# shayneobrien/generative-models

Measured on AMD Instinct MI355X. Metric: images/sec (28x28 MNIST) per D+G step, NSGAN bs=256, higher is better.
Workload: dtype f32; 1 GPU; NSGAN MNIST bs=256 fp32 per GPU (BASELINE.json configs[1]); 784-400-20 MLPs, N=50000 synthetic Bernoulli images, parity-mode RNG protocol, Adam 2e-4, D_steps=1; global_batch=256, parallelism=dp1, ranks_seen=1, gradient_exchange=none (1 rank), timing=one 2064-step timed region, cold_start_inclusive=False

## Files before the change

generative_models_amd/_lib.py:

```python
import ctypes
import os
from ctypes import POINTER, c_char_p, c_float, c_int, c_int32, c_int64, c_void_p

HERE = os.path.dirname(os.path.abspath(__file__))
LIB_PATH = os.environ.get("GM_LIB_PATH") or os.path.join(HERE, "libgm_hip.so")

GM_EINVAL = -10001
ACT_ID, ACT_RELU, ACT_SIGMOID = 0, 1, 2
ACT = {"id": ACT_ID, None: ACT_ID, "relu": ACT_RELU, "sigmoid": ACT_SIGMOID}
LOSS = {"ns": 0, "mm": 1, "w": 2, "ls": 3, "ra": 4, "fisher": 5, "f_total_variation": 6,
        "f_forward_kl": 7, "f_reverse_kl": 8, "f_pearson": 9, "f_hellinger": 10,
        "f_jensen_shannon": 11}


class Slot(ctypes.Structure):
    _fields_ = [("ctr", c_void_p), ("mul", c_int32), ("add", c_int32), ("ring", c_int32),
                ("stride", c_int64)]


def slot(ctr=0, mul=0, add=0, ring=0, stride=0):
    return Slot(ctr or None, mul, add, ring, stride)


NO_SLOT = Slot(None, 0, 0, 0, 0)
# ... 145 lines not shown
    "gm_version": (c_int, []),
    "gm_arch": (c_char_p, []),
    "gm_last_error": (c_char_p, []),
    "gm_tick": (c_int, [_P, _P, c_int64]),
    "gm_copy_slot_f32": (c_int, [_P, _P, Slot, _P, Slot, c_int64]),
    "gm_gather_rows": (c_int, [_P, _P, c_int64, _P, Slot, _P, c_int64, c_int, c_int]),
    "gm_linear_fwd": (c_int, [_P, _P, c_int64, Slot, _P, _P, _P, c_int64, c_int, c_int, c_int,
                              c_int]),
    "gm_linear_bwd_dx": (c_int, [_P, _P, c_int64, _P, _P, c_int64, _P, c_int64, c_int, c_int,
                                 c_int, c_int]),
    "gm_linear_bwd_dw": (c_int, [_P, _P, c_int64, _P, c_int64, Slot, _P, _P, c_int, c_int, c_int,
                                 c_int]),
    "gm_linear_fwd_ex": (c_int, [_P, POINTER(FwdArgs)]),
    "gm_linear_bwd_dx_ex": (c_int, [_P, POINTER(DxArgs)]),
    "gm_linear_bwd_dw_ex": (c_int, [_P, POINTER(DwAdamArgs), POINTER(DwAdamArgs), POINTER(DwTail)]),
    "gm_gan_loss": (c_int, [_P, c_int, c_int, _P, _P, c_int, c_int, POINTER(c_float), c_int,
                            c_float, _P, Slot, _P, _P, _P, _P]),
    "gm_gan_loss_phase": (c_int, [_P, c_int, c_int, _P, _P, c_int, c_int, POINTER(c_float), c_int,
                                  c_float, _P, Slot, _P, _P, _P, _P, c_int, _P, c_float]),
    "gm_l1_rows_dp": (c_int, [_P, _P, c_int64, _P, c_int64, c_int, c_int, c_int, c_int, _P, _P, c_int64, _P]),
    "gm_began_dloss_dp": (c_int, [_P, _P, c_int, c_int, _P, _P, Slot]),
    "gm_std_sums": (c_int, [_P, _P, c_int64, c_int, c_int, _P, _P]),
    "gm_std_from_sums": (c_int, [_P, _P, c_int64, _P]),
    "gm_adam": (c_int, [_P, _P, _P, _P, _P, c_int64, _P, Slot, ctypes.c_double, ctypes.c_double,
                        ctypes.c_double, ctypes.c_double, c_float]),
    "gm_interp": (c_int, [_P, _P, Slot, _P, c_int64, _P, c_int64, _P, c_int64, c_int, c_int]),
    "gm_gp_u": (c_int, [_P, _P, _P, c_int64, _P, _P, c_int64, c_int, c_int]),
    "gm_gp_norm": (c_int, [_P, _P, c_int64, _P, c_int64, _P, c_float, c_float, c_float, c_int,
                           c_int]),
    "gm_gp_dw2": (c_int, [_P, _P, _P, c_int64, _P, c_int64, _P, c_int, c_int]),
# ... 165 lines not shown
```

generative_models_amd/csrc/gm_gemm.hip:

```cpp
#include "gm_common.h"
#include "gm_head.h"
#include "gm_gather.h"
#include "gm_dvae.h"
#include "gm_ldsdma.h"

#include <cstdlib>
#include <type_traits>

typedef float f32x16 __attribute__((ext_vector_type(16)));

#ifdef GM_STAMPS
namespace gm_stamps {
constexpr int WAVES = 16, IDS = 40, HDR = 8, MAXB = 512, SLOT_WORDS = HDR + 2 * MAXB + WAVES * IDS * 2, SLOTS = 64;
static unsigned long long* host_buf = nullptr;
static int host_tile = 0, host_next = 0;
struct Ctx { unsigned long long* slot; int tile; };
__device__ __forceinline__ void rec(const Ctx& c, int tile, int id) {
    if (!c.slot || tile != c.tile || (threadIdx.x & 63)) return;
    __builtin_amdgcn_sched_barrier(0);
    unsigned long long* w = c.slot + HDR + 2 * MAXB + ((threadIdx.x >> 6) * IDS + id) * 2;
    w[0] = clock64(); w[1] = wall_clock64();
    __builtin_amdgcn_sched_barrier(0);
}
__device__ __forceinline__ void edge(const Ctx& c, bool exit_, int tile, int M, int N, int K, int mode) {
// ... 23 lines not shown
#define GM_STAMP_EDGE(p, exit_, tile, mode) do {} while (0)
#define GM_STAMP_AFTER(v) do {} while (0)
#endif

namespace {

constexpr int TM = 32, TN = 32;

enum { MODE_FWD = 0, MODE_DX = 1, MODE_DW = 2 };

struct GemmP {
    const float* A;
    const float* B;
    float* C;
    int M, N, K;
    int64_t lda, ldb, ldc;
    const float* bias;
    const float* aux;
    int64_t ldaux;
    float* db;
    int ones_from;
    int n_real;
    int epi;
    int accumulate;
    gm_slot a_slot, b_slot;
    int tn;
    int lds_tm, lds_mpx;
    int dma;
    int vec_epi;
    const float* ip_eps; gm_slot ip_slot;
    const float* ip_x; int64_t ip_ldx;
    float* ip_out; int64_t ip_ldo;
    int ip_rows;
    gm_adam_epi adam;
    const float* hd_w2; const float* hd_b2; float* hd_part; int64_t hd_ldp; float* hd_snap;
    const float* sq_x; int64_t sq_ldx; float* sq_dA; int64_t sq_lda; float* sq_part; int64_t sq_ldp;
    const float* rp_ml; int64_t rp_ldml; const float* rp_eps; gm_slot rp_slot; float* rp_dml; int64_t rp_ldd;
    int rp_Z;
    const float* fold_w2;
    const float* add;
    int64_t ldadd;
// ... 41 lines not shown
                                         int kb, int K) {
    const float* col = P + min(x, X - 1);
    return make_float4(col[(int64_t)min(kb + 0, K - 1) * ld], col[(int64_t)min(kb + 1, K - 1) * ld],
                       col[(int64_t)min(kb + 2, K - 1) * ld], col[(int64_t)min(kb + 3, K - 1) * ld]);
}
__device__ __forceinline__ float4 fix_xc(float4 v, int x, int X, int kb, int K, int ones_col,
                                         int ones_from = 0) {
    const bool okx = x < X, oc = (x == ones_col);
    v.x = (kb + 0 < K) ? (okx ? v.x : ((oc && kb + 0 >= ones_from) ? 1.f : 0.f)) : 0.f;
    v.y = (kb + 1 < K) ? (okx ? v.y : ((oc && kb + 1 >= ones_from) ? 1.f : 0.f)) : 0.f;
    v.z = (kb + 2 < K) ? (okx ? v.z : ((oc && kb + 2 >= ones_from) ? 1.f : 0.f)) : 0.f;
    v.w = (kb + 3 < K) ? (okx ? v.w : ((oc && kb + 3 >= ones_from) ? 1.f : 0.f)) : 0.f;
    return v;
}

__device__ __forceinline__ float fwd_value(const GemmP& p, float v, int n) {
    if (p.bias) v += p.bias[n];
    if (p.epi == GM_ACT_RELU) v = fmaxf(v, 0.f);
    else if (p.epi == GM_ACT_SIGMOID) v = gm_sigmoid(v);
    return v;
}

template <int MODE, bool LBL = false>
__device__ __forceinline__ void store_element(const GemmP& p, float v, int m, int n, float* kept = nullptr) {
    if (MODE == MODE_FWD) {
        if constexpr (LBL) v += p.lb_E[(int64_t)n * p.lb_C + gm_row_label(p.lb, m, p.lb_C)];
        v = fwd_value(p, v, n);
        p.C[(int64_t)m * p.ldc + n] = v;
        if (p.ip_out && m < p.ip_rows) {
            const float ev = (p.ip_eps + gm_slot_offset(p.ip_slot))[m];
// ... 567 lines not shown
#pragma unroll
                for (int f = 0; f < NI; ++f)
#pragma unroll
                    for (int r = 0; r < 4; ++r) {
                        const int row = MI * (4 * g4 + r) + e, col = NI * i16 + f;
                        if ((row >> 5) == bm && (col >> 5) == bnk)
                            red[red_idx(w, row & 31, col & 31)] = acc[e][f][r];
                    }
            __syncthreads();
            reduce_and_store<MODE_DW, WAVES, (MI > 1 ? 32 : 16)>(p, red, t, m0 + 32 * bm, n0 + 32 * bnk,
                                                                 (2 * bnk + 1 < NI) ? 0x7fffffff : n0 + 32 * bnk + 16,
                                                                 (2 * bm + 1 < MI) ? 32 : 16);
        }
}

template <int MI, int NI, bool OF, int FOLD, bool SL>
__device__ __forceinline__ void gemm16_dw_dma(const GemmP& p, float* red, int bx, int by, float* sds,
                                              const FoldP* fold, int gx) {
    constexpr int WAVES = 16, NP = MI + NI, CH = NP * 256;
    if (gx > 0) {
        const int gy = (p.M + 16 * MI - 1) / (16 * MI), total = gx * gy;
        const int L = by * gx + bx, x = L & 7, k = L >> 3;
        const int base = total >> 3, rem = total & 7;
        const int T = x * base + min(x, rem) + k;
        by = T % gy; bx = T / gy;
    }
    const int t = threadIdx.x, lane = t & 63;
    const int w = __builtin_amdgcn_readfirstlane(t >> 6);
    const int i16 = lane & 15, g4 = lane >> 4;
    const int m0 = by * (16 * MI), n0 = bx * (16 * NI);
#ifdef GM_STAMPS
    const gm_stamps::Ctx st_slot = p.stamp; const int st_tile = by * max(gx, 1) + bx;
#endif
    GM_STAMP_EDGE(p, false, st_tile, MODE_DW + 20);
    GM_STAMP(st_slot, st_tile, 0);
    const int b_cols = p.n_real;
    const int ones_col = p.db ? p.n_real : -1;
    const int nchunks = (p.K + 15) >> 4;
    float* buf = red + w * CH;
    const uint32_t buf_b = (uint32_t)(uintptr_t)buf;
    const int am = m0 + MI * i16, bn = n0 + NI * i16;

    const float* src[NP]; int srow[NP], sld[NP];
#pragma unroll
    for (int j = 0; j < NP; ++j) {
        const bool isA = j < MI;
        const int idx = (isA ? j : j - MI) * 64 + lane;
        const int row = isA ? idx / (4 * MI) : idx / (4 * NI);
        const int c4 = isA ? idx % (4 * MI) : idx % (4 * NI);
        const int col = isA ? min(m0 + 4 * c4, p.M - 4) : min(n0 + 4 * c4, b_cols - 4);
        src[j] = (isA ? slot_base<SL>(p.A, p.a_slot) : slot_base<SL>(p.B, p.b_slot)) + col;
        sld[j] = isA ? (int)p.lda : (int)p.ldb;
        srow[j] = row;
    }
    auto issue = [&](int c) {
#pragma unroll
        for (int j = 0; j < NP; ++j) {
            const int k = min(16 * c + srow[j], p.K - 1);
            slab::glds16(src[j] + (int64_t)k * sld[j], buf_b + j * 1024u);
        }
    };

    float fw[FOLD == 1 ? MI : 1];
    if constexpr (FOLD == 1) {
#pragma unroll
        for (int e = 0; e < MI; ++e) fw[e] = (am + e < p.M) ? p.fold_w2[min(am + e, p.M - 1)] : 0.f;
    }
// ... 58 lines not shown
    GM_STAMP(st_slot, st_tile, 9);
    dw_il_reduce<MI, NI>(p, red, acc, m0, n0, true);
    GM_STAMP(st_slot, st_tile, 12);
    GM_STAMP_EDGE(p, true, st_tile, MODE_DW + 20);
}

template <int MODE, bool DMA, int MI, int NI> struct RedSize {
    static constexpr int base = 16 * 32 * 32;
    static constexpr int onepass = (MODE == MODE_DW && MI * NI > 4) ? 16 * 256 * MI * NI : 0;
    static constexpr int dma = (MODE == MODE_DW && DMA) ? 16 * (MI + NI) * 256 : 0;
    static constexpr int m1 = base > onepass ? base : onepass;
    static constexpr int value = m1 > dma ? m1 : dma;
};

template <int MODE, bool VEC, int WAVES, int G, bool XV, int MI, int NI, bool OF = false, int FOLD = 0, bool DMA = false,
          bool TP = false, bool PK = false, bool SL = true, bool LBL = false>
__device__ __forceinline__ void gemm16_body(const GemmP& p, float* red, int bx, int by,
                                            float* sds = nullptr, const FoldP* fold = nullptr, int gx = 0,
                                            float* kept = nullptr) {
    static_assert(!TP || (FOLD == 1 && !DMA), "two-phase losses: folded weight gradient, operands through registers");
    static_assert(FOLD == 0 || (FOLD == 1 && MODE == MODE_DW && XV) || (FOLD == 2 && MODE == MODE_DX && VEC),
                  "folded head: 16-byte operand paths only");
    static_assert(G == 1, "per-chunk schedule (G stays in the kernel names so that they keep their shape across rounds)");
    static_assert(!PK || (WAVES == 16 && !DMA && ((MODE == MODE_FWD && VEC) || (MODE == MODE_DW && XV))),
                  "bit-packed operand rows: 16-byte operand paths through registers only");
    if constexpr (DMA && MODE == MODE_DW && XV && WAVES == 16 && FOLD != 2) {
        gemm16_dw_dma<MI, NI, OF, FOLD, SL>(p, red, bx, by, sds, fold, gx);
        return;
    }
    const int t = threadIdx.x;
    const int lane = t & 63, w = t >> 6;
    const int i16 = lane & 15, g4 = lane >> 4;
    const int m0 = by * (16 * MI), n0 = bx * (16 * NI);
#ifdef GM_STAMPS
    const gm_stamps::Ctx st_slot = p.stamp; const int st_tile = by * (int)gridDim.x + bx;
#endif
    GM_STAMP_EDGE(p, false, st_tile, MODE);
    GM_STAMP(st_slot, st_tile, 0);

    const float* A = slot_base<SL>(p.A, p.a_slot);
    const float* B = slot_base<SL>(p.B, p.b_slot);
    const int b_cols = (MODE == MODE_DW) ? p.n_real : p.N;
    const int ones_col = (MODE == MODE_DW && p.db) ? p.n_real : -1;
    const int nchunks = (p.K + 15) >> 4;
    GM_STAMP_AFTER(A); GM_STAMP_AFTER(B); GM_STAMP_AFTER(nchunks);
    GM_STAMP(st_slot, st_tile, 16);

    float4 fw[FOLD == 1 ? MI : 1];
    float fds[FOLD == 2 ? MI : 1];
    const int xq_ld = lane & 3, xe_ld = (lane >> 2) & 3;
    constexpr bool XMAP_A = MODE == MODE_DW && XV, XMAP_B = MODE != MODE_FWD && XV;
    const int ia = XMAP_A ? sigma16(i16) : i16, ib = XMAP_B ? sigma16(i16) : i16;
    if constexpr (FOLD == 1) {
#pragma unroll
        for (int mi = 0; mi < MI; ++mi)
            fw[mi] = *reinterpret_cast<const float4*>(
                p.fold_w2 + min(m0 + 16 * mi + 4 * xq_ld, p.M - 4));
    }
    auto load_a = [&](int c, int mi) -> float4 {
        const int kb = 16 * c + 4 * g4, x0 = m0 + 16 * mi;
        if (MODE == MODE_DW) {
            if (XV) return raw_xc4_16(A, p.lda, x0, p.M, c, p.K, lane);
            return raw_xc(A, p.lda, x0 + i16, p.M, kb, p.K);
        }
        return raw_kc<VEC>(A, p.lda, x0 + i16, p.M, kb, p.K);
    };
    auto load_b = [&](int c, int ni) -> float4 {
        const int kb = 16 * c + 4 * g4, x0 = n0 + 16 * ni;
        if (MODE == MODE_FWD) return raw_kc<VEC>(B, p.ldb, x0 + i16, p.N, kb, p.K);
        if (XV) return raw_xc4_16(B, p.ldb, x0, b_cols, c, p.K, lane);
        return raw_xc(B, p.ldb, x0 + i16, b_cols, kb, p.K);
    };
    auto fix_a = [&](float4 v, int c, int mi, float4 wk) -> float4 {
        const int kb = 16 * c + 4 * g4, x = m0 + 16 * mi + ia;
        if constexpr (FOLD == 1)
            v = fold_dh4(v, sds[min(16 * c + 4 * g4 + xe_ld, p.K - 1)], fw[mi]);
        if constexpr (FOLD == 2) v = fold_dh4(v, fds[mi], wk);
        if (MODE == MODE_DW)
            return fix_xc(XV ? lane48_transpose(v, lane) : v, x, p.M, kb, p.K, -1);
        return fix_kc(v, x, p.M, kb, p.K);
    };
    auto fix_b = [&](float4 v, int c, int ni) -> float4 {
        const int kb = 16 * c + 4 * g4, x = n0 + 16 * ni + ib;
        if (MODE == MODE_FWD) return fix_kc(v, x, p.N, kb, p.K);
        return fix_xc(XV ? lane48_transpose(v, lane) : v, x, b_cols, kb, p.K, ones_col, OF ? p.ones_from : 0);
    };

    f32x4 acc[MI][NI];
#pragma unroll
    for (int mi = 0; mi < MI; ++mi)
#pragma unroll
        for (int ni = 0; ni < NI; ++ni) acc[mi][ni] = f32x4{0.f, 0.f, 0.f, 0.f};

    const int nq = (nchunks - w + WAVES - 1) / WAVES;
    auto consume = [&](const float4 (&ra)[MI], const float4 (&rb)[NI], float4 wk, int q) {
        const int cq = w + q * WAVES;
        float4 fa[MI], fb[NI];
#pragma unroll
        for (int mi = 0; mi < MI; ++mi) fa[mi] = fix_a(ra[mi], cq, mi, wk);
#pragma unroll
        for (int ni = 0; ni < NI; ++ni) fb[ni] = fix_b(rb[ni], cq, ni);
        GM_STAMP_AFTER(fa[MI - 1].x); GM_STAMP_AFTER(fb[NI - 1].x);
        if (q < 4) GM_STAMP(st_slot, st_tile, 1 + 2 * q);
#pragma unroll
        for (int mi = 0; mi < MI; ++mi)
#pragma unroll
            for (int ni = 0; ni < NI; ++ni) {
                f32x4 c4 = acc[mi][ni];
                c4 = __builtin_amdgcn_mfma_f32_16x16x4f32(fa[mi].x, fb[ni].x, c4, 0, 0, 0);
                c4 = __builtin_amdgcn_mfma_f32_16x16x4f32(fa[mi].y, fb[ni].y, c4, 0, 0, 0);
// ... 33 lines not shown
            }
        } else if constexpr (FOLD == 2) {
            if (t < 16 * MI) {
                float s_, ds_, l_;
                fold_row(*fold, min(m0 + t, fold->R - 1), s_, ds_, l_);
                sds[t] = ds_;
            }
            GM_STAMP(st_slot, st_tile, 15);
            __syncthreads();
#pragma unroll
            for (int mi = 0; mi < MI; ++mi) fds[mi] = sds[16 * mi + i16];
        }
    };
    if constexpr (PK) {
        constexpr int PN = MODE == MODE_FWD ? MI : NI;
        auto pk_elem = [&](int c, int j) -> int {
            return MODE == MODE_FWD ? min(16 * c + 4 * g4, p.K - 4) : min(n0 + 16 * j + 4 * xq_ld, b_cols - 4);
        };
        auto load_pk = [&](int c, int j) -> uint32_t {
            const int row = MODE == MODE_FWD ? m0 + 16 * j + i16 : 16 * c + 4 * g4 + xe_ld;
            return p.pk_bits[(int64_t)row * p.pk_wpr + (pk_elem(c, j) >> 5)];
        };
        const int nq_s = __builtin_amdgcn_readfirstlane(nq);
        int q_pk;
        if (MODE == MODE_FWD) q_pk = (m0 < p.pk_rows) ? nq_s : 0;
        else q_pk = min(nq_s, max(0, ((p.pk_rows >> 4) - __builtin_amdgcn_readfirstlane(w) + WAVES - 1) / WAVES));
        auto do_chunk = [&](auto is_pk, auto with_prologue, int q) {
            constexpr bool P = decltype(is_pk)::value;
            float4 ra[MI], rb[NI];
            uint32_t pw[PN];
// ... 38 lines not shown
        float4 pv[4];
        if constexpr (FOLD == 1 && !TP) {
            if (t < fold->R) fold_part_load(*fold, t, pv);
        }
        if constexpr (FOLD == 2) {
            if (t < 16 * MI) fold_part_load(*fold, min(m0 + t, fold->R - 1), pv);
        }
        if (have) {
#pragma unroll
            for (int mi = 0; mi < MI; ++mi) ra[mi] = load_a(w, mi);
#pragma unroll
            for (int ni = 0; ni < NI; ++ni) rb[ni] = load_b(w, ni);
            wk = load_wk(w);
        }
        GM_STAMP(st_slot, st_tile, 17);
        if constexpr (FOLD == 1 && !TP) fold_fill_lds_pre(*fold, sds, fold->R, pv);
        else if constexpr (FOLD == 2) {
            if (t < 16 * MI) {
                float s_, ds_, l_;
                fold_row_of(*fold, min(m0 + t, fold->R - 1), fold_score_of(*fold, pv), s_, ds_, l_);
                sds[t] = ds_;
            }
            GM_STAMP(st_slot, st_tile, 15);
            __syncthreads();
#pragma unroll
            for (int mi = 0; mi < MI; ++mi) fds[mi] = sds[16 * mi + i16];
        }
        else fold_prologue();
        GM_STAMP(st_slot, st_tile, 13);
        if (have) consume(ra, rb, wk, 0);
        q_first = 1;
    }
    for (int q = q_first; q < nq; ++q) {
        float4 ra[MI], rb[NI];
        const int cc = w + q * WAVES;
#pragma unroll
        for (int mi = 0; mi < MI; ++mi) ra[mi] = load_a(cc, mi);
#pragma unroll
        for (int ni = 0; ni < NI; ++ni) rb[ni] = load_b(cc, ni);
        const float4 wk = load_wk(cc);
        consume(ra, rb, wk, q);
    }
    }
    GM_STAMP(st_slot, st_tile, 9);
    if constexpr (MODE == MODE_DW && WAVES == 16 && MI * NI > 4) {
// ... 26 lines not shown
            if (bm + bn == 0) GM_STAMP(st_slot, st_tile, 10);
            reduce_and_store<MODE, WAVES, (MI > 1 ? 32 : 16), LBL>(p, red, t, m0 + 32 * bm, n0 + 32 * bn,
                                                              (2 * bn + 1 < NI) ? 0x7fffffff : n0 + 32 * bn + 16,
                                                              (2 * bm + 1 < MI) ? 32 : 16,
                                                              kept ? kept + 32 * bm * KEEP_LD + 32 * bn : nullptr);
        }
    GM_STAMP(st_slot, st_tile, 12);
    GM_STAMP_EDGE(p, true, st_tile, MODE);
}

template <int MODE, bool VEC, int WAVES, int G, bool XV, int MI, int NI, bool DMA = false, bool SL = false>
__global__ __launch_bounds__(WAVES * 64) void gemm16_kernel(GemmP p) {
    __shared__ __attribute__((aligned(16))) float red[(WAVES == 16) ? RedSize<MODE, DMA, MI, NI>::value : WAVES * 32 * 32];
    gemm16_body<MODE, VEC, WAVES, G, XV, MI, NI, false, 0, DMA, false, false, SL>(p, red, blockIdx.x, blockIdx.y, nullptr, nullptr,
                                                                                  (int)gridDim.x);
}

template <bool VEC, int MI, int NI>
__global__ __launch_bounds__(1024) void gemm16_fwd_label_kernel(GemmP p) {
    __shared__ __attribute__((aligned(16))) float red[RedSize<MODE_FWD, false, MI, NI>::value];
    gemm16_body<MODE_FWD, VEC, 16, 1, false, MI, NI, false, 0, false, false, false, false, true>(p, red, blockIdx.x, blockIdx.y,
                                                                                                nullptr, nullptr, (int)gridDim.x);
}

template <int MODE, bool VEC, int G, bool XV, int MI, int NI, bool OF = false, bool FOLDED = false, bool DMA = false,
          bool TP = false, bool PK = false>
__device__ __forceinline__ void gemm16_with_head(const GemmP& p, const HeadBwdP& hp, int hrows,
                                                 int hblocks) {
    __shared__ __attribute__((aligned(16))) float red[RedSize<MODE, DMA, MI, NI>::value];
    __shared__ float sds[FOLDED ? FOLD_MAX_ROWS : 1];
// ... 264 lines not shown
}

template <int MODE>
int vec_epi_ok(const GemmP& p) {
    if (!aligned16(p.C) || p.ldc % 4 != 0) return 0;
    if (MODE == MODE_FWD) {
        if (p.bias && !aligned16(p.bias)) return 0;
        if (p.ip_out && !(aligned16(p.ip_out) && aligned16(p.ip_x) && p.ip_ldo % 4 == 0 && p.ip_ldx % 4 == 0)) return 0;
    } else if (MODE == MODE_DX) {
        if (p.epi != GM_ACT_ID && !(aligned16(p.aux) && p.ldaux % 4 == 0)) return 0;
        if (p.add && !(aligned16(p.add) && p.ldadd % 4 == 0)) return 0;
    } else {
        if (p.adam.enabled && !(aligned16(p.adam.pW) && aligned16(p.adam.mW) && aligned16(p.adam.vW))) return 0;
    }
    return 1;
}

struct Rider {
    const HeadBwdP* head = nullptr;
    const GatherP* gather = nullptr;
    const CorruptP* corrupt = nullptr;
    const GemmP* pair = nullptr;
    bool pair_xvec = false;
    const gm_fin2* fin = nullptr;
    const L1RideP* l1 = nullptr;
};

inline void launch_gather_alone(hipStream_t s, const Rider& r) {
    const GatherP& gp = *r.gather;
    if (r.corrupt)
// ... 49 lines not shown
#endif
    const bool xv = xvec && MODE != MODE_FWD;
    const bool slots = has_slot(p.a_slot) || has_slot(p.b_slot);
    if (slots && (folded || p.pk_bits)) {
        gm_set_error("ring slots on the operands of a folded-head / bit-packed launch are not supported");
        return GM_EINVAL;
    }
    const bool ride_head = head && !slots;
    auto dma_ok = [&](const GemmP& q, bool qxv) {
        constexpr int dma_min_k = 768;
        return MODE == MODE_DW && qxv && q.K >= dma_min_k && q.M >= 4 && q.n_real >= 4 &&
               ((int64_t)q.K + 64) * (q.lda > q.ldb ? q.lda : q.ldb) < (1ll << 31);
    };
    p.dma = dma_ok(p, xv);
    if (p.pk_bits) {
        if constexpr (MODE == MODE_FWD) {
            if (!vec || !p.hd_part || rider.gather || p.ip_out) {
                gm_set_error("bit-packed rows: the forward needs 16-byte aligned operands and the folded head's partial dots");
                return GM_EINVAL;
            }
            const dim3 bgrid((p.N + 31) / 32, (p.M + 31) / 32);
            hipLaunchKernelGGL(gemm16_fwd_bits_kernel, bgrid, dim3(1024), 0, s, p);
            GM_LAUNCH_RET();
        } else if constexpr (MODE == MODE_DW) {
            if (!head || !folded || head->fold.enabled != 1 || !xv || p.ones_from > 0 || rider.pair) {
                gm_set_error("bit-packed rows: the weight gradient needs the folded head of a separable loss and "
                             "16-byte aligned operands");
                return GM_EINVAL;
            }
            p.dma = false;
            const dim3 bgrid((p.N + 47) / 48, (p.M + 31) / 32);
            const int hblocks = gm_head_bwd_blocks(*head);
            const int hrows = (hblocks + (int)bgrid.x - 1) / (int)bgrid.x;
            hipLaunchKernelGGL(gemm16_dw_head_bits_kernel, dim3(bgrid.x, bgrid.y + hrows), dim3(1024), 0, s, p, *head,
                               hrows, hblocks);
            GM_LAUNCH_RET();
        } else {
            gm_set_error("bit-packed rows: forward and weight gradient only");
            return GM_EINVAL;
        }
    }
    if constexpr (MODE != MODE_DW) {
        if (!rider.pair && !folded && !p.hd_part && !p.sq_part && !slots) {
            const int cfg = lds_cfg_for<MODE>(p, vec, xv);
            if (cfg) {
                if (head) hipLaunchKernelGGL(head_bwd_kernel, dim3(gm_head_bwd_blocks(*head)), dim3(1024), 0, s, *head);
                if (rider.gather) launch_gather_alone(s, rider);
                return launch_lds<MODE>(s, p, cfg);
// ... 12 lines not shown
                const int gblocks = gm_gather_blocks(gp, 4);
                const int grows = (gblocks + (int)kgrid.x - 1) / (int)kgrid.x;
                const dim3 ggrid(kgrid.x, kgrid.y + grows);
                if (slots) hipLaunchKernelGGL((gemm16_k32_fwd_kernel<true, true>), ggrid, dim3(256), 0, s, p, gp, grows, gblocks);
                else hipLaunchKernelGGL((gemm16_k32_fwd_kernel<false, true>), ggrid, dim3(256), 0, s, p, gp, grows, gblocks);
            } else {
                if (slots) hipLaunchKernelGGL((gemm16_k32_fwd_kernel<true, false>), kgrid, dim3(256), 0, s, p, GatherP{}, 0, 0);
                else hipLaunchKernelGGL((gemm16_k32_fwd_kernel<false, false>), kgrid, dim3(256), 0, s, p, GatherP{}, 0, 0);
            }
            GM_LAUNCH_RET();
        }
    }
    const int tile = pick_tile<MODE>(p);
    const int mi = tile_mi(tile), ni = tile_ni(tile);
    const dim3 grid((p.N + 16 * ni - 1) / (16 * ni), (p.M + 16 * mi - 1) / (16 * mi));
    if constexpr (MODE == MODE_DW) {
        if (ride_head) {
            const int hblocks = gm_head_bwd_blocks(*head);
            const int hrows = (hblocks + (int)grid.x - 1) / (int)grid.x;
            const dim3 hgrid(grid.x, grid.y + hrows);
            if (folded && (!xv || p.ones_from > 0)) {
                gm_set_error("folded head: the weight gradient needs 16-byte aligned operands and no stacked rows");
                return GM_EINVAL;
            }
#define GM_LH(X, OFV, FD) GM_TILE_SWITCH(tile, p.dma && (X), GM_LH1_##X##_##OFV##_##FD)
#define GM_LHK(X, OFV, FD, MI_, NI_, D_) hipLaunchKernelGGL((gemm16_dw_head_kernel<false, 1, X, MI_, NI_, OFV, FD, ((X) && (D_))>), hgrid, dim3(1024), 0, s, p, *head, hrows, hblocks)
#define GM_LH1_true_false_true(MI_, NI_, D_) GM_LHK(true, false, true, MI_, NI_, D_)
#define GM_LH1_true_true_false(MI_, NI_, D_) GM_LHK(true, true, false, MI_, NI_, D_)
#define GM_LH1_true_false_false(MI_, NI_, D_) GM_LHK(true, false, false, MI_, NI_, D_)
#define GM_LH1_false_true_false(MI_, NI_, D_) GM_LHK(false, true, false, MI_, NI_, D_)
// ... 86 lines not shown
                r2.l1 = nullptr;
                const int rc = launch<MODE_DW>(s, p_in, vec, xvec, r2);
                if (rc) return rc;
                const L1RideP& l = *rider.l1;
                GemmP f{};
                f.A = l.z; f.B = pb.adam.pW; f.C = l.H; f.M = l.rows; f.N = pb.M; f.K = pb.n_real;
                f.lda = l.ldz; f.ldb = pb.ldc; f.ldc = l.ldh; f.bias = pb.adam.pb; f.epi = GM_ACT_RELU;
                f.a_slot = l.z_slot; f.b_slot = gm_slot{};
                const bool fvec = aligned16(l.z) && aligned16(pb.adam.pW) && (l.ldz % 4 == 0) && (f.K % 4 == 0) &&
                                  (pb.ldc % 4 == 0) && (l.z_slot.stride % 4 == 0);
                return launch<MODE_FWD>(s, f, fvec);
            }
            if (pairable) {
                const bool dma = p.dma && dma_ok(pb, true);
                p.dma = pb.dma = dma;
                const int tna = (int)grid.x, na = (int)(grid.x * grid.y);
                if (l1_rides) {
                    const dim3 lgrid(na + (pb.M + 15) / 16);
#define GM_LL1(MI_, NI_, D_) hipLaunchKernelGGL((gemm16_dw_pair_l1_kernel<MI_, NI_>), lgrid, dim3(1024), 0, s, p, pb, na, tna, *rider.l1)
                    GM_TILE_SWITCH(tile, false, GM_LL1);
#undef GM_LL1
                    GM_LAUNCH_RET();
                }
                const int tnb = (pb.N + 16 * ni - 1) / (16 * ni), tmb = (pb.M + 16 * mi - 1) / (16 * mi);
                const dim3 pgrid(na + tnb * tmb);
                const bool sl_b = has_slot(pb.a_slot) || has_slot(pb.b_slot);
#define GM_LP2(K_, GRID_, MI_, NI_, D_, ...)                                                                              \
    do {                                                                                                                  \
        if (slots) hipLaunchKernelGGL((K_<1, true, MI_, NI_, D_, true, true>), GRID_, dim3(1024), 0, s, __VA_ARGS__);     \
        else if (sl_b) hipLaunchKernelGGL((K_<1, true, MI_, NI_, D_, false, true>), GRID_, dim3(1024), 0, s, __VA_ARGS__); \
// ... 125 lines not shown
    } else if (label) {
        GM_CHECK_ARG(a.lb_E && a.lb.labels && a.lb_C > 0 && a.lb_C <= 32);
        p.lb = a.lb; p.lb_E = a.lb_E; p.lb_C = a.lb_C;
        return fwd_label_launch((hipStream_t)stream, p, vec);
    } else if (a.gather) {
        const float* gout = nullptr;
        const int rc = gather_from_args(*a.gather, true, &g, &c, &r.corrupt, &gout);
        if (rc) return rc;
        GM_CHECK_ARG(gout != a.Y && gout != a.X);
        GM_CHECK_ARG(!r.corrupt || (c.out_c != a.Y && (const float*)c.out_c != a.X));
        r.gather = &g;
    }
    return launch<MODE_FWD>((hipStream_t)stream, p, vec, false, r);
}

static int fwd_label_launch(hipStream_t s, const GemmP& p, bool vec) {
    const int tile = pick_tile<MODE_FWD>(p);
    const dim3 grid((p.N + 16 * tile_ni(tile) - 1) / (16 * tile_ni(tile)), (p.M + 16 * tile_mi(tile) - 1) / (16 * tile_mi(tile)));
#define GM_LBL(MI_, NI_, D_)                                                                                \
    do {                                                                                                    \
        if (vec) hipLaunchKernelGGL((gemm16_fwd_label_kernel<true, MI_, NI_>), grid, dim3(1024), 0, s, p);  \
        else hipLaunchKernelGGL((gemm16_fwd_label_kernel<false, MI_, NI_>), grid, dim3(1024), 0, s, p);     \
    } while (0)
    GM_TILE_SWITCH(tile, false, GM_LBL);
#undef GM_LBL
    GM_LAUNCH_RET();
}

extern "C" int gm_linear_fwd(void* stream, const float* X, int64_t ldx, gm_slot x_slot, const float* W,
                             const float* bias, float* Y, int64_t ldy, int M, int K, int N, int act) {
    gm_fwd_args a{};
    a.X = X; a.ldx = ldx; a.x_slot = x_slot; a.W = W; a.bias = bias; a.Y = Y; a.ldy = ldy;
// ... 172 lines not shown
    rc = dw_fill(b, &pb, &xb);
    if (rc) return rc;
    r.pair = &pb;
    r.pair_xvec = xb;
    return launch<MODE_DW>((hipStream_t)stream, pa, false, xa, r);
}

extern "C" int gm_linear_bwd_dw(void* stream, const float* dA, int64_t lda, const float* X, int64_t ldx,
                                gm_slot x_slot, float* dW, float* db, int M, int K, int N, int accumulate) {
    gm_dw_adam_args a{};
    a.dA = dA; a.lda = lda; a.X = X; a.ldx = ldx; a.x_slot = x_slot; a.dW = dW; a.db = db;
    a.M = M; a.K = K; a.N = N; a.accumulate = accumulate;
    return dw_impl(stream, &a, nullptr, nullptr);
}

extern "C" int gm_linear_bwd_dw_ex(void* stream, const gm_dw_adam_args* first, const gm_dw_adam_args* second,
                                   const gm_dw_tail* tail) {
    return dw_impl(stream, first, second, tail);
}
```

include/gm_hip.h:

```cpp
#ifndef GM_HIP_H
#define GM_HIP_H

#include <stddef.h>
#include <stdint.h>

#ifdef __cplusplus
extern "C" {
#endif

#define GM_EINVAL (-10001)

enum { GM_ACT_ID = 0, GM_ACT_RELU = 1, GM_ACT_SIGMOID = 2 };

enum {
    GM_LOSS_NS = 0,
    GM_LOSS_MM = 1,
    GM_LOSS_W = 2,
    GM_LOSS_LS = 3,
    GM_LOSS_RA = 4,
    GM_LOSS_FISHER = 5,
    GM_LOSS_F_TV = 6, GM_LOSS_F_FKL = 7, GM_LOSS_F_RKL = 8, GM_LOSS_F_PEARSON = 9,
    GM_LOSS_F_HELLINGER = 10, GM_LOSS_F_JS = 11
};

// ... 382 lines not shown
    const gm_head_bwd_args* head; const gm_head_fold_args* fold;
    const uint32_t* xbits; int xbits_wpr, xbits_rows;
} gm_dw_adam_args;
typedef struct gm_finalize2_args {
    const float* pa; int na; float scale_a; float* out_a; gm_slot slot_a;
    const float* pb; int nb; float scale_b; float* out_b; gm_slot slot_b;
    int64_t* tick; unsigned int* done;
} gm_finalize2_args;
typedef struct gm_dw_tail {
    const float* z; int64_t ldz; gm_slot z_slot; float* H; int64_t ldh; int rows;
    const gm_finalize2_args* fin;
} gm_dw_tail;
int gm_linear_bwd_dw_ex(void* stream, const gm_dw_adam_args* first, const gm_dw_adam_args* second,
                        const gm_dw_tail* tail);

int gm_pdw_couple(void* stream, const float* x, int64_t ldx, const float* xr, int64_t ldr, const float* t,
                  gm_slot t_slot, float* n, float* share, float* dA, int64_t ldd, float* xhat, int64_t ldh,
                  float* xcopy, int64_t ldc, float inv_b, int B, int I);
int gm_pdw_dir(void* stream, const float* g, int64_t ldg, const float* x, int64_t ldx, const float* xr, int64_t ldr,
               const float* n, float* gamma, int64_t ldm, float* pen, float lambda, float inv_b, int B, int I);

#define GM_IWAE_TAG_TRAIN 0x49574145u
#define GM_IWAE_TAG_EVAL 0x49574556u
#define GM_IWAE_MAX_K 64
#define GM_IWAE_MAX_Z 32
typedef struct gm_iwae_noise {
    uint64_t seed;
    uint32_t tag;
    const int64_t* step_ctr;
    const int64_t* step_base;
// ... 35 lines not shown
```

Before: 4.195 million images/sec.

## Use 32-bit byte offsets and precomputed row offsets in GEMM operand loads

Adds a near-addressing path in which per-row byte offsets for the A and B operands are precomputed once as 32-bit values, and the leading dimensions, chunk count, column count and ones column are packed host-side into GemmP fields. This cuts 64-bit address arithmetic and repeated index math in the inner load loops. Small tiles also issue their first operand loads before zeroing the accumulators, to hide load latency. Operands reaching past 2^32 bytes fall back to a separate far kernel, which adds another template instantiation and host-side checks.

```diff
diff --git a/generative_models_amd/_lib.py b/generative_models_amd/_lib.py
--- a/generative_models_amd/_lib.py
+++ b/generative_models_amd/_lib.py
@@ -183,6 +183,8 @@
     "gm_linear_fwd_ex": (c_int, [_P, POINTER(FwdArgs)]),
     "gm_linear_bwd_dx_ex": (c_int, [_P, POINTER(DxArgs)]),
     "gm_linear_bwd_dw_ex": (c_int, [_P, POINTER(DwAdamArgs), POINTER(DwAdamArgs), POINTER(DwTail)]),
+    "gm_gemm_operand_reach": (c_int, [c_int, c_int, c_int, c_int, c_int64, c_int64, c_int,
+                                      POINTER(ctypes.c_uint64)]),
     "gm_gan_loss": (c_int, [_P, c_int, c_int, _P, _P, c_int, c_int, POINTER(c_float), c_int,
                             c_float, _P, Slot, _P, _P, _P, _P]),
     "gm_gan_loss_phase": (c_int, [_P, c_int, c_int, _P, _P, c_int, c_int, POINTER(c_float), c_int,
diff --git a/generative_models_amd/csrc/gm_gemm.hip b/generative_models_amd/csrc/gm_gemm.hip
--- a/generative_models_amd/csrc/gm_gemm.hip
+++ b/generative_models_amd/csrc/gm_gemm.hip
@@ -61,7 +61,9 @@
     const float* B;
     float* C;
     int M, N, K;
-    int64_t lda, ldb, ldc;
+    union { int64_t lda; struct { uint32_t a_ldb; int nchunks; }; };
+    union { int64_t ldb; struct { uint32_t b_ldb; int b_cols; }; };
+    int64_t ldc;
     const float* bias;
     const float* aux;
     int64_t ldaux;
@@ -71,7 +73,7 @@
     int epi;
     int accumulate;
     gm_slot a_slot, b_slot;
-    int tn;
+    union { int tn; int ones_col; };
     int lds_tm, lds_mpx;
     int dma;
     int vec_epi;
@@ -143,6 +145,23 @@
     return v;
 }
 
+__device__ __forceinline__ float4 near4(const float* __restrict__ P, uint32_t off) {
+    return *reinterpret_cast<const float4*>(reinterpret_cast<const char*>(P) + off);
+}
+__device__ __forceinline__ float near1(const float* __restrict__ P, uint32_t off) {
+    return *reinterpret_cast<const float*>(reinterpret_cast<const char*>(P) + off);
+}
+template <bool VEC>
+__device__ __forceinline__ float4 near_kc(const float* __restrict__ P, uint32_t rowoff, int kb, int K) {
+    if (VEC) return near4(P, rowoff + 4u * (uint32_t)min(kb, K - 4));
+    return make_float4(near1(P, rowoff + 4u * (uint32_t)min(kb + 0, K - 1)), near1(P, rowoff + 4u * (uint32_t)min(kb + 1, K - 1)),
+                       near1(P, rowoff + 4u * (uint32_t)min(kb + 2, K - 1)), near1(P, rowoff + 4u * (uint32_t)min(kb + 3, K - 1)));
+}
+__device__ __forceinline__ float4 near_xc(const float* __restrict__ P, uint32_t stride, uint32_t xoff, int kb, int K) {
+    return make_float4(near1(P, (uint32_t)min(kb + 0, K - 1) * stride + xoff), near1(P, (uint32_t)min(kb + 1, K - 1) * stride + xoff),
+                       near1(P, (uint32_t)min(kb + 2, K - 1) * stride + xoff), near1(P, (uint32_t)min(kb + 3, K - 1) * stride + xoff));
+}
+
 __device__ __forceinline__ float fwd_value(const GemmP& p, float v, int n) {
     if (p.bias) v += p.bias[n];
     if (p.epi == GM_ACT_RELU) v = fmaxf(v, 0.f);
@@ -740,7 +759,7 @@
         }
 }
 
-template <int MI, int NI, bool OF, int FOLD, bool SL>
+template <int MI, int NI, bool OF, int FOLD, bool SL, bool FAR = false>
 __device__ __forceinline__ void gemm16_dw_dma(const GemmP& p, float* red, int bx, int by, float* sds,
                                               const FoldP* fold, int gx) {
     constexpr int WAVES = 16, NP = MI + NI, CH = NP * 256;
@@ -761,8 +780,8 @@
     GM_STAMP_EDGE(p, false, st_tile, MODE_DW + 20);
     GM_STAMP(st_slot, st_tile, 0);
     const int b_cols = p.n_real;
-    const int ones_col = p.db ? p.n_real : -1;
-    const int nchunks = (p.K + 15) >> 4;
+    const int ones_col = FAR ? (p.db ? p.n_real : -1) : p.ones_col;
+    const int nchunks = FAR ? (p.K + 15) >> 4 : p.nchunks;
     float* buf = red + w * CH;
     const uint32_t buf_b = (uint32_t)(uintptr_t)buf;
     const int am = m0 + MI * i16, bn = n0 + NI * i16;
@@ -776,7 +795,8 @@
         const int c4 = isA ? idx % (4 * MI) : idx % (4 * NI);
         const int col = isA ? min(m0 + 4 * c4, p.M - 4) : min(n0 + 4 * c4, b_cols - 4);
         src[j] = (isA ? slot_base<SL>(p.A, p.a_slot) : slot_base<SL>(p.B, p.b_slot)) + col;
-        sld[j] = isA ? (int)p.lda : (int)p.ldb;
+        if constexpr (FAR) sld[j] = isA ? (int)p.lda : (int)p.ldb;
+        else sld[j] = isA ? (int)(p.a_ldb >> 2) : (int)(p.b_ldb >> 2);
         srow[j] = row;
     }
     auto issue = [&](int c) {
@@ -865,7 +885,7 @@
 };
 
 template <int MODE, bool VEC, int WAVES, int G, bool XV, int MI, int NI, bool OF = false, int FOLD = 0, bool DMA = false,
-          bool TP = false, bool PK = false, bool SL = true, bool LBL = false>
+          bool TP = false, bool PK = false, bool SL = true, bool LBL = false, bool FAR = false>
 __device__ __forceinline__ void gemm16_body(const GemmP& p, float* red, int bx, int by,
                                             float* sds = nullptr, const FoldP* fold = nullptr, int gx = 0,
                                             float* kept = nullptr) {
@@ -876,7 +896,7 @@
     static_assert(!PK || (WAVES == 16 && !DMA && ((MODE == MODE_FWD && VEC) || (MODE == MODE_DW && XV))),
                   "bit-packed operand rows: 16-byte operand paths through registers only");
     if constexpr (DMA && MODE == MODE_DW && XV && WAVES == 16 && FOLD != 2) {
-        gemm16_dw_dma<MI, NI, OF, FOLD, SL>(p, red, bx, by, sds, fold, gx);
+        gemm16_dw_dma<MI, NI, OF, FOLD, SL, FAR>(p, red, bx, by, sds, fold, gx);
         return;
     }
     const int t = threadIdx.x;
@@ -891,9 +911,9 @@
 
     const float* A = slot_base<SL>(p.A, p.a_slot);
     const float* B = slot_base<SL>(p.B, p.b_slot);
-    const int b_cols = (MODE == MODE_DW) ? p.n_real : p.N;
-    const int ones_col = (MODE == MODE_DW && p.db) ? p.n_real : -1;
-    const int nchunks = (p.K + 15) >> 4;
+    const int b_cols = FAR ? ((MODE == MODE_DW) ? p.n_real : p.N) : p.b_cols;
+    const int ones_col = FAR ? ((MODE == MODE_DW && p.db) ? p.n_real : -1) : p.ones_col;
+    const int nchunks = FAR ? (p.K + 15) >> 4 : p.nchunks;
     GM_STAMP_AFTER(A); GM_STAMP_AFTER(B); GM_STAMP_AFTER(nchunks);
     GM_STAMP(st_slot, st_tile, 16);
 
@@ -908,19 +928,48 @@
             fw[mi] = *reinterpret_cast<const float4*>(
                 p.fold_w2 + min(m0 + 16 * mi + 4 * xq_ld, p.M - 4));
     }
-    auto load_a = [&](int c, int mi) -> float4 {
+    uint32_t oa[MI], ob[NI];
+    if constexpr (!FAR) {
+#pragma unroll
+        for (int mi = 0; mi < MI; ++mi) {
+            const int x0 = m0 + 16 * mi;
+            if (MODE == MODE_DW) oa[mi] = 4u * (uint32_t)(XV ? min(x0 + 4 * xq_ld, p.M - 4) : min(x0 + i16, p.M - 1));
+            else oa[mi] = (uint32_t)min(x0 + i16, p.M - 1) * p.a_ldb;
+        }
+#pragma unroll
+        for (int ni = 0; ni < NI; ++ni) {
+            const int x0 = n0 + 16 * ni;
+            if (MODE == MODE_FWD) ob[ni] = (uint32_t)min(x0 + i16, p.N - 1) * p.b_ldb;
+            else ob[ni] = 4u * (uint32_t)(XV ? min(x0 + 4 * xq_ld, b_cols - 4) : min(x0 + i16, b_cols - 1));
+        }
+    }
+    auto load_a = [&](int c, int mi) __attribute__((always_inline)) -> float4 {
         const int kb = 16 * c + 4 * g4, x0 = m0 + 16 * mi;
-        if (MODE == MODE_DW) {
-            if (XV) return raw_xc4_16(A, p.lda, x0, p.M, c, p.K, lane);
-            return raw_xc(A, p.lda, x0 + i16, p.M, kb, p.K);
-        }
-        return raw_kc<VEC>(A, p.lda, x0 + i16, p.M, kb, p.K);
+        if constexpr (!FAR) {
+            if (MODE == MODE_DW) {
+                if (XV) return near4(A, (uint32_t)min(kb + xe_ld, p.K - 1) * p.a_ldb + oa[mi]);
+                return near_xc(A, p.a_ldb, oa[mi], kb, p.K);
+            }
+            return near_kc<VEC>(A, oa[mi], kb, p.K);
+        } else {
+            if (MODE == MODE_DW) {
+                if (XV) return raw_xc4_16(A, p.lda, x0, p.M, c, p.K, lane);
+                return raw_xc(A, p.lda, x0 + i16, p.M, kb, p.K);
+            }
+            return raw_kc<VEC>(A, p.lda, x0 + i16, p.M, kb, p.K);
+        }
     };
-    auto load_b = [&](int c, int ni) -> float4 {
+    auto load_b = [&](int c, int ni) __attribute__((always_inline)) -> float4 {
         const int kb = 16 * c + 4 * g4, x0 = n0 + 16 * ni;
-        if (MODE == MODE_FWD) return raw_kc<VEC>(B, p.ldb, x0 + i16, p.N, kb, p.K);
-        if (XV) return raw_xc4_16(B, p.ldb, x0, b_cols, c, p.K, lane);
-        return raw_xc(B, p.ldb, x0 + i16, b_cols, kb, p.K);
+        if constexpr (!FAR) {
+            if (MODE == MODE_FWD) return near_kc<VEC>(B, ob[ni], kb, p.K);
+            if (XV) return near4(B, (uint32_t)min(kb + xe_ld, p.K - 1) * p.b_ldb + ob[ni]);
+            return near_xc(B, p.b_ldb, ob[ni], kb, p.K);
+        } else {
+            if (MODE == MODE_FWD) return raw_kc<VEC>(B, p.ldb, x0 + i16, p.N, kb, p.K);
+            if (XV) return raw_xc4_16(B, p.ldb, x0, b_cols, c, p.K, lane);
+            return raw_xc(B, p.ldb, x0 + i16, b_cols, kb, p.K);
+        }
     };
     auto fix_a = [&](float4 v, int c, int mi, float4 wk) -> float4 {
         const int kb = 16 * c + 4 * g4, x = m0 + 16 * mi + ia;
@@ -938,13 +987,15 @@
     };
 
     f32x4 acc[MI][NI];
-#pragma unroll
-    for (int mi = 0; mi < MI; ++mi)
-#pragma unroll
-        for (int ni = 0; ni < NI; ++ni) acc[mi][ni] = f32x4{0.f, 0.f, 0.f, 0.f};
+    auto zero_acc = [&]() __attribute__((always_inline)) {
+#pragma unroll
+        for (int mi = 0; mi < MI; ++mi)
+#pragma unroll
+            for (int ni = 0; ni < NI; ++ni) acc[mi][ni] = f32x4{0.f, 0.f, 0.f, 0.f};
+    };
 
     const int nq = (nchunks - w + WAVES - 1) / WAVES;
-    auto consume = [&](const float4 (&ra)[MI], const float4 (&rb)[NI], float4 wk, int q) {
+    auto consume = [&](const float4 (&ra)[MI], const float4 (&rb)[NI], float4 wk, int q) __attribute__((always_inline)) {
         const int cq = w + q * WAVES;
         float4 fa[MI], fb[NI];
 #pragma unroll
@@ -1008,6 +1059,7 @@
     };
     if constexpr (PK) {
         constexpr int PN = MODE == MODE_FWD ? MI : NI;
+        zero_acc();
         auto pk_elem = [&](int c, int j) -> int {
             return MODE == MODE_FWD ? min(16 * c + 4 * g4, p.K - 4) : min(n0 + 16 * j + 4 * xq_ld, b_cols - 4);
         };
@@ -1076,6 +1128,8 @@
             wk = load_wk(w);
         }
         GM_STAMP(st_slot, st_tile, 17);
+        __builtin_amdgcn_sched_barrier(0);
+        zero_acc();
         if constexpr (FOLD == 1 && !TP) fold_fill_lds_pre(*fold, sds, fold->R, pv);
         else if constexpr (FOLD == 2) {
             if (t < 16 * MI) {
@@ -1091,6 +1145,19 @@
         else fold_prologue();
         GM_STAMP(st_slot, st_tile, 13);
         if (have) consume(ra, rb, wk, 0);
+        q_first = 1;
+    } else if constexpr (MI * NI > 6 || (MI == 1 && NI == 4)) {
+        zero_acc();
+    } else {
+        float4 ra[MI], rb[NI];
+#pragma unroll
+        for (int mi = 0; mi < MI; ++mi) ra[mi] = load_a(w, mi);
+#pragma unroll
+        for (int ni = 0; ni < NI; ++ni) rb[ni] = load_b(w, ni);
+        GM_STAMP(st_slot, st_tile, 17);
+        __builtin_amdgcn_sched_barrier(0);
+        zero_acc();
+        if (nq > 0) consume(ra, rb, make_float4(0.f, 0.f, 0.f, 0.f), 0);
         q_first = 1;
     }
     for (int q = q_first; q < nq; ++q) {
@@ -1147,6 +1214,13 @@
     __shared__ __attribute__((aligned(16))) float red[(WAVES == 16) ? RedSize<MODE, DMA, MI, NI>::value : WAVES * 32 * 32];
     gemm16_body<MODE, VEC, WAVES, G, XV, MI, NI, false, 0, DMA, false, false, SL>(p, red, blockIdx.x, blockIdx.y, nullptr, nullptr,
                                                                                   (int)gridDim.x);
+}
+
+template <int MODE, bool VEC, int WAVES, int G, bool XV, int MI, int NI, bool DMA = false>
+__global__ __launch_bounds__(WAVES * 64) void gemm16_far_kernel(GemmP p) {
+    __shared__ __attribute__((aligned(16))) float red[(WAVES == 16) ? RedSize<MODE, DMA, MI, NI>::value : WAVES * 32 * 32];
+    gemm16_body<MODE, VEC, WAVES, G, XV, MI, NI, false, 0, DMA, false, false, false, false, true>(
+        p, red, blockIdx.x, blockIdx.y, nullptr, nullptr, (int)gridDim.x);
 }
 
 template <bool VEC, int MI, int NI>
@@ -1441,6 +1515,27 @@
         if (p.adam.enabled && !(aligned16(p.adam.pW) && aligned16(p.adam.mW) && aligned16(p.adam.vW))) return 0;
     }
     return 1;
+}
+
+template <int MODE>
+void operand_reach(const GemmP& p, uint64_t* ra, uint64_t* rb) {
+    const uint64_t M = (uint64_t)p.M, N = (uint64_t)p.N, K = (uint64_t)p.K, la = (uint64_t)p.lda, lb = (uint64_t)p.ldb;
+    const uint64_t bc = (MODE == MODE_DW) ? (uint64_t)p.n_real : N;
+    *ra = 4 * ((MODE == MODE_DW) ? (K - 1) * la + M : (M - 1) * la + K);
+    *rb = 4 * ((MODE == MODE_FWD) ? (N - 1) * lb + K : (K - 1) * lb + bc);
+}
+template <int MODE>
+bool operands_near(const GemmP& p) {
+    uint64_t ra, rb;
+    operand_reach<MODE>(p, &ra, &rb);
+    return ra <= (1ull << 32) && rb <= (1ull << 32);
+}
+template <int MODE>
+void near_pack(GemmP& p) {
+    const int64_t la = p.lda, lb = p.ldb;
+    p.a_ldb = (uint32_t)((uint64_t)la * 4); p.nchunks = (p.K + 15) >> 4;
+    p.b_ldb = (uint32_t)((uint64_t)lb * 4); p.b_cols = (MODE == MODE_DW) ? p.n_real : p.N;
+    p.ones_col = (MODE == MODE_DW && p.db) ? p.n_real : -1;
 }
 
 struct Rider {
@@ -1520,12 +1615,17 @@
     };
     p.dma = dma_ok(p, xv);
     if (p.pk_bits) {
+        if (!operands_near<MODE>(p)) {
+            gm_set_error("bit-packed rows: an operand reaches 2^32 bytes past its base");
+            return GM_EINVAL;
+        }
         if constexpr (MODE == MODE_FWD) {
             if (!vec || !p.hd_part || rider.gather || p.ip_out) {
                 gm_set_error("bit-packed rows: the forward needs 16-byte aligned operands and the folded head's partial dots");
                 return GM_EINVAL;
             }
             const dim3 bgrid((p.N + 31) / 32, (p.M + 31) / 32);
+            near_pack<MODE>(p);
             hipLaunchKernelGGL(gemm16_fwd_bits_kernel, bgrid, dim3(1024), 0, s, p);
             GM_LAUNCH_RET();
         } else if constexpr (MODE == MODE_DW) {
@@ -1538,6 +1638,7 @@
             const dim3 bgrid((p.N + 47) / 48, (p.M + 31) / 32);
             const int hblocks = gm_head_bwd_blocks(*head);
             const int hrows = (hblocks + (int)bgrid.x - 1) / (int)bgrid.x;
+            near_pack<MODE>(p);
             hipLaunchKernelGGL(gemm16_dw_head_bits_kernel, dim3(bgrid.x, bgrid.y + hrows), dim3(1024), 0, s, p, *head,
                                hrows, hblocks);
             GM_LAUNCH_RET();
@@ -1580,6 +1681,27 @@
     const int tile = pick_tile<MODE>(p);
     const int mi = tile_mi(tile), ni = tile_ni(tile);
     const dim3 grid((p.N + 16 * ni - 1) / (16 * ni), (p.M + 16 * mi - 1) / (16 * mi));
+    if (!operands_near<MODE>(p) || (MODE == MODE_DW && rider.pair && !operands_near<MODE_DW>(*rider.pair))) {
+        if (head || rider.gather || rider.pair || slots) {
+            gm_set_error("an operand reaches 2^32 bytes past its base: plain launches without riders or ring slots only");
+            return GM_EINVAL;
+        }
+#define GM_LFAR(V, X, MI_, NI_, D_) \
+    hipLaunchKernelGGL((gemm16_far_kernel<MODE, V, 16, 1, X, MI_, NI_, (MODE == MODE_DW && (X) && (D_))>), grid, dim3(1024), 0, s, p)
+#define GM_LFAR_tt(MI_, NI_, D_) GM_LFAR(true, true, MI_, NI_, D_)
+#define GM_LFAR_tf(MI_, NI_, D_) GM_LFAR(true, false, MI_, NI_, D_)
+#define GM_LFAR_ft(MI_, NI_, D_) GM_LFAR(false, true, MI_, NI_, D_)
+#define GM_LFAR_ff(MI_, NI_, D_) GM_LFAR(false, false, MI_, NI_, D_)
+        if (xv) { if (vec) GM_TILE_SWITCH(tile, p.dma, GM_LFAR_tt); else GM_TILE_SWITCH(tile, p.dma, GM_LFAR_ft); }
+        else    { if (vec) GM_TILE_SWITCH(tile, false, GM_LFAR_tf); else GM_TILE_SWITCH(tile, false, GM_LFAR_ff); }
+#undef GM_LFAR_ff
+#undef GM_LFAR_ft
+#undef GM_LFAR_tf
+#undef GM_LFAR_tt
+#undef GM_LFAR
+        GM_LAUNCH_RET();
+    }
+    near_pack<MODE>(p);
     if constexpr (MODE == MODE_DW) {
         if (ride_head) {
             const int hblocks = gm_head_bwd_blocks(*head);
@@ -1696,6 +1818,7 @@
             if (pairable) {
                 const bool dma = p.dma && dma_ok(pb, true);
                 p.dma = pb.dma = dma;
+                near_pack<MODE_DW>(pb);
                 const int tna = (int)grid.x, na = (int)(grid.x * grid.y);
                 if (l1_rides) {
                     const dim3 lgrid(na + (pb.M + 15) / 16);
@@ -1851,8 +1974,14 @@
     return launch<MODE_FWD>((hipStream_t)stream, p, vec, false, r);
 }
 
-static int fwd_label_launch(hipStream_t s, const GemmP& p, bool vec) {
+static int fwd_label_launch(hipStream_t s, const GemmP& p_in, bool vec) {
+    GemmP p = p_in;
+    if (!operands_near<MODE_FWD>(p)) {
+        gm_set_error("class-conditional forward: an operand reaches 2^32 bytes past its base");
+        return GM_EINVAL;
+    }
     const int tile = pick_tile<MODE_FWD>(p);
+    near_pack<MODE_FWD>(p);
     const dim3 grid((p.N + 16 * tile_ni(tile) - 1) / (16 * tile_ni(tile)), (p.M + 16 * tile_mi(tile) - 1) / (16 * tile_mi(tile)));
 #define GM_LBL(MI_, NI_, D_)                                                                                \
     do {                                                                                                    \
@@ -2055,6 +2184,19 @@
     return dw_impl(stream, &a, nullptr, nullptr);
 }
 
+extern "C" int gm_gemm_operand_reach(int kind, int M, int K, int N, int64_t ld_rows, int64_t ld_second, int with_db,
+                                     unsigned long long* reach2) {
+    GM_CHECK_ARG(kind >= 0 && kind <= 2 && M > 0 && K > 0 && N > 0 && ld_rows > 0 && ld_second > 0 && reach2);
+    GemmP p{};
+    uint64_t ra, rb;
+    p.lda = ld_rows; p.ldb = ld_second;
+    if (kind == MODE_FWD) { p.M = M; p.N = N; p.K = K; operand_reach<MODE_FWD>(p, &ra, &rb); }
+    else if (kind == MODE_DX) { p.M = M; p.N = K; p.K = N; operand_reach<MODE_DX>(p, &ra, &rb); }
+    else { p.M = N; p.N = K + (with_db ? 1 : 0); p.K = M; p.n_real = K; operand_reach<MODE_DW>(p, &ra, &rb); }
+    reach2[0] = ra; reach2[1] = rb;
+    return (ra <= (1ull << 32) && rb <= (1ull << 32)) ? 1 : 0;
+}
+
 extern "C" int gm_linear_bwd_dw_ex(void* stream, const gm_dw_adam_args* first, const gm_dw_adam_args* second,
                                    const gm_dw_tail* tail) {
     return dw_impl(stream, first, second, tail);
diff --git a/include/gm_hip.h b/include/gm_hip.h
--- a/include/gm_hip.h
+++ b/include/gm_hip.h
@@ -420,6 +420,9 @@
 int gm_linear_bwd_dw_ex(void* stream, const gm_dw_adam_args* first, const gm_dw_adam_args* second,
                         const gm_dw_tail* tail);
 
+int gm_gemm_operand_reach(int kind, int M, int K, int N, int64_t ld_rows, int64_t ld_second, int with_db,
+                          unsigned long long* reach2);
+
 int gm_pdw_couple(void* stream, const float* x, int64_t ldx, const float* xr, int64_t ldr, const float* t,
                   gm_slot t_slot, float* n, float* share, float* dA, int64_t ldd, float* xhat, int64_t ldh,
                   float* xcopy, int64_t ldc, float inv_b, int B, int I);
```

Result: no change. 4.205 million images/sec, median of 3 (+0.2%).
